# DiltheyLab/MetaMaps

Hardware: AMD Instinct MI355X
Metric: Gbp long reads mapped+classified per sec (whole node), miniSeq+H DB (higher is better)
Workload: dtype u32

## Files before the change

### include/metamaps_hip.h

```cpp
#ifndef METAMAPS_HIP_H
#define METAMAPS_HIP_H

#include <stddef.h>
#include <stdint.h>

#ifdef __cplusplus
extern "C" {
#endif

#define MM_ABI_VERSION 6

typedef enum {
  MM_OK = 0,
  MM_ERR_ARG = -1,
  MM_ERR_DEVICE = -2,
  MM_ERR_NOMEM = -3,
  MM_ERR_STATE = -4,
  MM_ERR_LIMIT = -5,
  MM_ERR_NUMERIC = -6,
  MM_ERR_COMM = -7,
  MM_ERR_DATA = -8
} mm_status;

typedef struct mm_ctx mm_ctx;
// ... 135 lines not shown
  double ms_minimizer, ms_sketch, ms_probe_gather, ms_sort_hits, ms_l1_scan, ms_l2, ms_compact, ms_total, ms_hit_filter;
  int64_t n_reads_giant;
} mm_map_stats;

int mm_map_batch(mm_ctx* ctx, const mm_index* idx, const mm_seqset* reads, const mm_map_params* p, mm_mapping** out);
int mm_map_batch_phased(mm_ctx* ctx, const mm_index* idx, const mm_seqset* reads, const mm_map_params* p, void (*at_stage)(void* user, int stage), void* user,
                        mm_mapping** out);
int mm_map_batch_reusing(mm_ctx* ctx, const mm_index* idx, const mm_seqset* reads, const mm_map_params* p, const mm_mapping* sketch_of, mm_mapping** out);
int mm_sketch_batch(mm_ctx* ctx, const mm_seqset* reads, const mm_map_params* p, mm_mapping** out);
void mm_mapping_destroy(mm_mapping* m);
int mm_mapping_get_stats(const mm_mapping* m, mm_map_stats* out);
int mm_mapping_release_intermediates(mm_mapping* m);
int mm_mapping_fetch(mm_mapping* m, int64_t* offsets, mm_map_record* records, int64_t cap);
int mm_mapping_add_qualities(mm_ctx* ctx, mm_mapping* m, const mm_seqset* reads, int k);
int mm_mapping_keep_best(mm_ctx* ctx, mm_mapping* m, int k);
int mm_mapping_concat(mm_ctx* ctx, mm_mapping* const* parts, const int32_t* contig_base, int n_parts, mm_mapping** out);
int mm_mapping_from_parts(mm_ctx* ctx, int64_t n_reads, const int32_t* read_len, const mm_map_params* p, int n_parts,
                          const int64_t* const* offsets, const mm_map_record* const* records, const int32_t* contig_base, mm_mapping** out);

int mm_mapping_gather(mm_ctx* ctx, int owner, int64_t n_reads, const int32_t* read_len, const mm_map_params* p, mm_mapping* const* parts, const int32_t* chunk_id,
                      int n_parts, int n_chunks, const int32_t* chunk_rank, const int32_t* contig_base, mm_mapping** out);

int mm_debug_sketch(mm_mapping* m, int64_t* offsets, uint32_t* hash, int32_t* strand, int64_t cap);
int mm_debug_hits(mm_mapping* m, int64_t* offsets, int32_t* contig, int32_t* wpos, int64_t cap);
int mm_debug_candidates(mm_mapping* m, int64_t* offsets, int32_t* triples , int64_t cap);
int mm_debug_l2(mm_mapping* m, int64_t* per_cand , int64_t cap);
int mm_debug_min_hits(mm_mapping* m, int32_t* min_hits );
int mm_debug_probed_lists(mm_mapping* m, const mm_index* idx, int64_t* hist, int32_t n_bins);

int mm_em_create(mm_ctx* ctx, int64_t n_reads, const int64_t* read_off, const int32_t* taxon, const double* mapq,
                 const double* inv_nloc, int32_t n_taxa, mm_em** out);
int mm_em_create_from_mapping(mm_ctx* ctx, const mm_mapping* m, const int32_t* contig_taxon, const int32_t* contig_len, int32_t n_contigs,
                              int32_t n_taxa, mm_em** out);
int mm_em_taxon_counts(mm_em* em, int64_t* counts);
int mm_em_sizes(const mm_em* em, int64_t* n_reads, int64_t* n_entries, int32_t* n_taxa);
void mm_em_destroy(mm_em* em);
int mm_em_iterate(mm_em* em, const double* f, double* f_partial, double* ll_partial);
int mm_em_iterate_allreduce(mm_em* em, const double* f, double* f_next, double* ll);
int mm_em_run(mm_em* em, const double* f0, int max_iter, double* f_out, double* ll_trace, int ll_cap, int* n_iter);
int mm_em_continue(mm_em* em, int max_iter, double* f_out, double* ll_trace, int ll_cap, int* n_iter, int* stopped);
int mm_em_posteriors(mm_em* em, const double* f, double* post , int64_t* best );
int mm_em_bootstrap(mm_em* em, const double* f_start, int32_t rep0, int32_t n_rep, uint64_t seed, const uint8_t* weights,
                    int max_iter, double* f_out, double* ll_out, int32_t* n_iter, int32_t* stopped);
int mm_em_lca(mm_em* em, const double* f, int32_t n_nodes, const int32_t* parent, const int32_t* taxon_node, double threshold,
              int32_t* node_out, double* mass_out, int64_t* direct_out);

// ... 27 lines not shown
```

### metamaps_amd/capi.py

```python
from __future__ import annotations

import ctypes as C
import os
import re

import numpy as np

_HERE = os.path.dirname(os.path.abspath(__file__))
LIB_PATH = os.path.join(_HERE, "csrc", "libmetamaps_hip.so")
HEADER_PATH = os.path.join(os.path.dirname(_HERE), "include", "metamaps_hip.h")

COMM_ID_BYTES = 128
MM_ERR_ARG = -1
MM_ERR_LIMIT = -5
MM_ERR_DATA = -8


class MMError(RuntimeError):
    def __init__(self, status: int, msg: str):
        super().__init__(f"libmetamaps_hip status {status}: {msg}")
        self.status = status


SEED_STAGE_CB = C.CFUNCTYPE(None, C.c_void_p, C.c_int)
# ... 119 lines not shown
            "mm_index_set_freq_threshold": (C.c_int, [vp, C.c_int]),
            "mm_index_entries": (C.c_int, [vp, vp, vp, vp, vp, i64]),
            "mm_index_dup_neighbours": (C.c_int, [vp, vp, vp, i64]),
            "mm_recommended_window": (C.c_int, [f64, C.c_int, f32, C.c_int, u64]),
            "mm_estimate_pvalue": (f64, [C.c_int, C.c_int, f32, C.c_int, u64]),
            "mm_min_hits_relaxed": (C.c_int, [C.c_int, C.c_int, f32]),
            "mm_identity": (None, [C.c_int, C.c_int, C.c_int, P(f32), P(f32)]),
            "mm_map_batch": (C.c_int, [vp, vp, vp, P(MapParams), P(vp)]),
            "mm_map_batch_phased": (C.c_int, [vp, vp, vp, P(MapParams), SEED_STAGE_CB, vp, P(vp)]),
            "mm_map_batch_reusing": (C.c_int, [vp, vp, vp, P(MapParams), vp, P(vp)]),
            "mm_sketch_batch": (C.c_int, [vp, vp, P(MapParams), P(vp)]),
            "mm_mapping_destroy": (None, [vp]),
            "mm_mapping_get_stats": (C.c_int, [vp, P(MapStats)]),
            "mm_comm_info": (C.c_int, [vp, C.POINTER(C.c_int), C.POINTER(C.c_int)]),
            "mm_mapping_gather": (C.c_int, [vp, C.c_int, i64, vp, vp, vp, vp, C.c_int, C.c_int, vp, vp, vp]),
            "mm_mapping_release_intermediates": (C.c_int, [vp]),
            "mm_mapping_fetch": (C.c_int, [vp, vp, vp, i64]),
            "mm_mapping_add_qualities": (C.c_int, [vp, vp, vp, C.c_int]),
            "mm_mapping_concat": (C.c_int, [vp, P(vp), vp, C.c_int, P(vp)]),
            "mm_mapping_keep_best": (C.c_int, [vp, vp, C.c_int]),
            "mm_mapping_from_parts": (C.c_int, [vp, i64, vp, P(MapParams), C.c_int, P(vp), P(vp), vp, P(vp)]),
            "mm_index_plan_chunks": (C.c_int, [vp, vp, u64, vp, i32, P(i32)]),
            "mm_debug_sketch": (C.c_int, [vp, vp, vp, vp, i64]),
            "mm_debug_hits": (C.c_int, [vp, vp, vp, vp, i64]),
            "mm_debug_candidates": (C.c_int, [vp, vp, vp, i64]),
            "mm_debug_l2": (C.c_int, [vp, vp, i64]),
            "mm_debug_min_hits": (C.c_int, [vp, vp]),
            "mm_debug_probed_lists": (C.c_int, [vp, vp, vp, i32]),
            "mm_em_create": (C.c_int, [vp, i64, vp, vp, vp, vp, i32, P(vp)]),
            "mm_em_create_from_mapping": (C.c_int, [vp, vp, vp, vp, i32, i32, P(vp)]),
            "mm_em_taxon_counts": (C.c_int, [vp, vp]),
            "mm_em_sizes": (C.c_int, [vp, P(i64), P(i64), P(i32)]),
            "mm_em_destroy": (None, [vp]),
            "mm_em_iterate": (C.c_int, [vp, vp, vp, P(f64)]),
            "mm_em_iterate_allreduce": (C.c_int, [vp, vp, vp, P(f64)]),
            "mm_em_posteriors": (C.c_int, [vp, vp, vp, vp]),
            "mm_em_run": (C.c_int, [vp, vp, C.c_int, vp, vp, C.c_int, P(C.c_int)]),
            "mm_em_continue": (C.c_int, [vp, C.c_int, vp, vp, C.c_int, P(C.c_int), P(C.c_int)]),
            "mm_em_bootstrap": (C.c_int, [vp, vp, i32, i32, u64, vp, C.c_int, vp, vp, vp, vp]),
            "mm_em_lca": (C.c_int, [vp, vp, i32, vp, vp, f64, vp, vp, vp]),
            "mm_gene_overlap": (C.c_int, [vp, i32, vp, vp, vp, vp, i32, vp, vp, i32, i64, vp, vp, vp, vp, vp, vp, vp, P(i64)]),
            "mm_ident_filter": (C.c_int, [vp, i64, vp, vp, vp, vp, i32, f64, vp, P(i64), P(i64), vp, vp, vp, vp, vp, vp, vp, P(i64), P(i64)]),
            "mm_comm_unique_id": (C.c_int, [C.c_char_p]),
            "mm_comm_init": (C.c_int, [vp, C.c_char_p, C.c_int, C.c_int]),
            "mm_comm_allreduce_f64": (C.c_int, [vp, vp, i64]),
            "mm_comm_share": (C.c_int, [vp, vp]),
            "mm_comm_destroy": (None, [vp]),
        }
        for name, (res, args) in sig.items():
            fn = getattr(L, name)
            fn.restype = res
            fn.argtypes = args
        _lib = L
    return _lib


def _ptr(a):
    return None if a is None else a.ctypes.data_as(C.c_void_p)


class Context:
    def __init__(self, device: int = 0):
        self.h = C.c_void_p()
        st = lib().mm_ctx_create(device, C.byref(self.h))
        if st != 0:
            raise MMError(st, "mm_ctx_create failed (no gfx950 GPU visible? this library has no CPU fallback)")

    def check(self, st: int):
        if st != 0:
            raise MMError(st, lib().mm_last_error(self.h).decode(errors="replace"))

    def close(self):
# ... 454 lines not shown
        arr = (C.c_void_p * max(len(parts), 1))(*[p.h for p in parts])
        cid = np.asarray(chunk_id, dtype=np.int32); crk = np.asarray(chunk_rank, dtype=np.int32); base = np.asarray(contig_base, dtype=np.int32)
        mp = MapParams(k, w, pi, min_read_len)
        out = C.c_void_p()
        ctx.check(lib().mm_mapping_gather(ctx.h, owner, len(rl), _ptr(rl), C.byref(mp), arr, _ptr(cid), len(parts), len(crk), _ptr(crk), _ptr(base), C.byref(out)))
        return Mapping(ctx, out, len(rl)) if out.value else None

    def fetch(self, rec_buf: np.ndarray | None = None):
        off = np.empty(self.n_reads + 1, dtype=np.int64)
        self.ctx.check(lib().mm_mapping_fetch(self.h, _ptr(off), None, 0))
        n = int(off[-1])
        rec = rec_buf[:n] if rec_buf is not None and len(rec_buf) >= n else np.empty(n, dtype=RECORD_DTYPE)
        self.ctx.check(lib().mm_mapping_fetch(self.h, _ptr(off), _ptr(rec), n))
        return off, rec

    def debug_sketch(self):
        off = np.zeros(self.n_reads + 1, dtype=np.int64)
        self.ctx.check(lib().mm_debug_sketch(self.h, _ptr(off), None, None, 0))
        h = np.zeros(int(off[-1]), dtype=np.uint32)
        s = np.zeros(int(off[-1]), dtype=np.int32)
        self.ctx.check(lib().mm_debug_sketch(self.h, _ptr(off), _ptr(h), _ptr(s), len(h)))
        return off, h, s

    def debug_hits(self):
        off = np.zeros(self.n_reads + 1, dtype=np.int64)
        self.ctx.check(lib().mm_debug_hits(self.h, _ptr(off), None, None, 0))
        c = np.zeros(int(off[-1]), dtype=np.int32)
        w = np.zeros(int(off[-1]), dtype=np.int32)
        self.ctx.check(lib().mm_debug_hits(self.h, _ptr(off), _ptr(c), _ptr(w), len(c)))
        return off, c, w

    def debug_candidates(self):
        off = np.zeros(self.n_reads + 1, dtype=np.int64)
        self.ctx.check(lib().mm_debug_candidates(self.h, _ptr(off), None, 0))
        t = np.zeros((int(off[-1]), 3), dtype=np.int32)
        self.ctx.check(lib().mm_debug_candidates(self.h, _ptr(off), _ptr(t), len(t)))
        return off, t

    def debug_l2(self, n_cand: int):
        a = np.zeros((n_cand, 6), dtype=np.int64)
        if n_cand:
            self.ctx.check(lib().mm_debug_l2(self.h, _ptr(a), n_cand))
        return a

    def debug_min_hits(self):
        a = np.zeros(self.n_reads, dtype=np.int32)
# ... 94 lines not shown
```

### metamaps_amd/csrc/mm_api.hip

```cpp
#include "mm_env.hpp"
#include "mm_map.hpp"
#include "mm_em.hpp"
#include "mm_stats.hpp"
#include "mm_synth.hpp"
#include "mm_hpc.hpp"
#include "mm_lca.hpp"
#include "mm_gene.hpp"
#include "mm_ident.hpp"
#include <chrono>
#include <new>
#include <rccl/rccl.h>
#include "mm_prims.hpp"

namespace mm {
void seqset_upload(mm_seqset* s);
void seqset_upload_nt16(mm_seqset* s);
int64_t bgzf_inflate(mm_ctx* ctx, const uint8_t* comp, int64_t comp_bytes, const int64_t* comp_off, const int32_t* comp_len, int32_t n,
                     uint8_t* out, int64_t out_cap, const int64_t* out_off, int32_t* status);
void bgzf_deflate(mm_ctx* ctx, const uint8_t* in, int64_t in_bytes, uint8_t* out, int64_t out_cap, int64_t* out_bytes, int32_t* n_blocks);
int64_t bgzf_deflate_bound(int64_t in_bytes);
mm_gzip* gzip_open(mm_ctx* ctx, int64_t chunk, int64_t segment);
void gzip_close(mm_gzip* g);
int gzip_feed(mm_gzip* g, const uint8_t* comp, int64_t n, bool last, int64_t* avail);
int64_t gzip_read(mm_gzip* g, uint8_t* out, int64_t cap);
// ... 748 lines not shown
  });
}

int mm_debug_sketch(mm_mapping* m, int64_t* offsets, uint32_t* hash, int32_t* strand, int64_t cap) {
  if (m && m->released) return MM_ERR_STATE;
  if (!m) return MM_ERR_ARG;
  return guarded(m->ctx, [&] {
    hipStream_t st = m->ctx->stream;
    int64_t tot = 0;
    for (int64_t r = 0; r < m->n_reads; ++r) { if (offsets) offsets[r] = tot; tot += m->h_sk_n[(size_t)r]; }
    if (offsets) offsets[m->n_reads] = tot;
    if (!hash && !strand) return;
    MM_REQUIRE(cap >= tot, MM_ERR_ARG, "output capacity too small");
    auto hh = m->sk_hash.to_host(st); auto hs = m->sk_strand.to_host(st);
    int64_t o = 0;
    for (int64_t r = 0; r < m->n_reads; ++r)
      for (int i = 0; i < m->h_sk_n[(size_t)r]; ++i, ++o) {
        size_t src = (size_t)m->mz.h_off[(size_t)r] + (size_t)i;
        if (hash) hash[o] = hh[src];
        if (strand) strand[o] = (hs[src] & 1) ? 1 : -1;
      }
  });
}
int mm_debug_hits(mm_mapping* m, int64_t* offsets, int32_t* contig, int32_t* wpos, int64_t cap) {
  if (m && m->released) return MM_ERR_STATE;
  if (!m) return MM_ERR_ARG;
  return guarded(m->ctx, [&] {
    const int64_t tot = (int64_t)m->h_read_hit_off[(size_t)m->n_reads];
    if (offsets) for (size_t i = 0; i < m->h_read_hit_off.size(); ++i) offsets[i] = (int64_t)m->h_read_hit_off[i];
    if (!contig && !wpos) return;
    MM_REQUIRE(cap >= tot, MM_ERR_ARG, "output capacity too small");
    auto h = m->hits.to_host(m->ctx->stream, (size_t)tot);
    for (int64_t i = 0; i < tot; ++i) {
      if (contig) contig[i] = (int32_t)(h[(size_t)i] >> 32);
      if (wpos) wpos[i] = mm::pw_wpos((uint32_t)h[(size_t)i]);
    }
  });
}
int mm_debug_candidates(mm_mapping* m, int64_t* offsets, int32_t* triples, int64_t cap) {
  if (m && m->released) return MM_ERR_STATE;
  if (!m) return MM_ERR_ARG;
  return guarded(m->ctx, [&] {
    if (offsets) for (size_t i = 0; i < m->h_cand_off.size(); ++i) offsets[i] = (int64_t)m->h_cand_off[i];
    if (!triples) return;
    MM_REQUIRE(cap >= m->n_cand, MM_ERR_ARG, "output capacity too small");
    m->cand.download(triples, (size_t)(3 * m->n_cand), m->ctx->stream);
// ... 169 lines not shown
```

### metamaps_amd/csrc/mm_env.hpp

```cpp
#pragma once
#include <unistd.h>
#include <cstdlib>
#include <cstring>
#include <string>

extern "C" char** environ;

namespace mm {

struct EnvSwitch { const char* name; const char* dflt; const char* kind; const char* what; };

inline const EnvSwitch* env_table(size_t* n) {
  static const EnvSwitch T[] = {
    {"MM_STRICT_ENV", "unset", "user", "refuse MM_* variables that are not in this table (mm_ctx_create returns MM_ERR_ARG, the CLI exits 1)"},
    {"MM_CPU_BUDGET", "min(hardware threads, affinity mask, cgroup CPU quota)", "user", "CPUs the process may keep busy: what every thread pool of the library and the CLI is sized from (cpu_budget.hpp)"},
    {"MM_SYNC", "block when the CPU budget is <= 32, else spin", "user", "how a host thread waits for its stream: \"spin\" (hipStreamSynchronize) or \"block\" (sleep on an event created with hipEventBlockingSync)"},
    {"MM_CLI_WORKERS", "4", "user", "worker contexts per GPU that take read batches in turn (= --workers-per-gpu)"},
    {"MM_CLI_BATCH_READS", "100000", "user", "reads per batch handed to a worker"},
    {"MM_CLI_BATCH_MBASES", "256", "user", "... or this many million bases, whichever comes first"},
    {"MM_CLI_MAP_SLOTS", "2", "tuning", "batches per device that may be inside their mapping section at the same time"},
    {"MM_CLI_BLOCK_BYTES", "128 MiB", "tuning", "block size of the block-parallel FASTQ/FASTA parser over an mmap-ed query file"},
    {"MM_CLI_REF_BLOCK_BYTES", "min(group, 256 MiB)", "tuning", "the same for the reference FASTA"},
    {"MM_CLI_REF_GROUP_BASES", "2^30", "test", "bases per upload group of the reference (small groups: the concat path on small inputs)"},
    {"MM_CLI_REF_SEQUENTIAL", "unset", "test", "reference through the sequential kseq-style reader instead of the block parser"},
// ... 6 lines not shown
    {"MM_DEFLATE_HOST", "unset", "test", "mm_bgzf_deflate (the mappings file of --compress-output) writes its BGZF members with zlib level 1 on the host's threads instead of the device kernel: the A/B partner and a fallback; other bytes, the same text"},
    {"MM_CLI_NO_PREWARM", "unset", "test", "worker contexts come up with their first batch instead of beside the index build"},
    {"MM_SF_GRID", "the device's CU count", "debug", "resident workgroups of the streaming seed filter (measurement aid: how K3 scales with the CUs at work)"},
    {"MM_CLI_LATE_READER", "unset", "debug", "the query reader starts when the index is built instead of beside the build (measurement aid)"},
    {"MM_CLI_NO_SKETCH_REUSE", "unset", "test", "chunk-major runs recompute minimizers and sketches per chunk (mm_map_batch instead of mm_map_batch_reusing)"},
    {"MM_CLI_NO_HUGE", "unset", "test", "no transparent-huge-page arena for host blocks >= 4 MiB (huge_new.hpp)"},
    {"MM_CLI_FULL_TEARDOWN", "unset", "test", "destroy every object and run static destructors at exit instead of _exit after the last file is closed"},
    {"MM_CLASSIFY_THREADS", "32", "user", "host threads that tokenise the mappings file and format classify's outputs"},
    {"MM_EM_MAX_ITER", "unbounded", "test", "cap on EM iterations in classify (the reference has none)"},
    {"MM_EM_SLICE", "1024", "test", "EM iterations per mm_em_run / mm_em_continue call of classify"},
    {"MM_CLI_TIMING", "unset", "debug", "phase laps of the CLI on stderr (bench.py's e2e legs parse them)"},
    {"MM_CLI_FORMAT_TRACE", "unset", "debug", "per-thread times of the text formatting of a batch on stderr"},
    {"MM_DEVICE_BYTES_CAP", "0 (off)", "test", "the library behaves as if every device had this many bytes: allocations beyond fail, mm_ctx_device_info reports it (placement tests)"},
    {"MM_INDEX_SCALE_MB", "8192", "test", "blocks from this size on are index-scale (pooled per device); a few MB exercise the pool on small inputs"},
    {"MM_NO_SLABS", "unset", "test", "worker buffers are not cut out of pooled index-scale blocks"},
    {"MM_NO_POOL_RESCUE", "unset", "test", "round-3 behaviour: a request the driver refuses hands the whole pool back instead of being served from it"},
    {"MM_ALLOC_TRACE", "unset", "debug", "every block that comes from the driver, with its cost, on stderr"},
    {"MM_CTX_TRACE", "unset", "debug", "phases of mm_ctx_create (HIP initialisation, stream, allocator) on stderr"},
    {"MM_HOST_TIMING", "unset", "debug", "host-side sections of mm_map_batch and of the index build on stderr"},
    {"MM_PACK_SCALAR", "unset", "test", "mm_seqset_upload packs bases with the byte-table loop only (cross-check of the AVX2 path, host_pack.cpp)"},
    {"MM_INDEX_PART_MAX", "2^31 - 2^24 entries", "test", "entries per partition of the hash sort (small values: the partitioned sort + merge on small inputs)"},
    {"MM_DUP_SAT", "65535", "test", "saturation value of the stored same-hash neighbour distances (small values: K5's scan fall-back)"},
    {"MM_EAGER_TIEBREAK", "unset", "test", "resolve every duplicate-hash strand by the reference's std::sort order up front instead of only where a strand vote reads one"},
    {"MM_FORCE_AMB_REDO", "unset", "test", "every read with an unresolved strand goes through the redo path"},
    {"MM_NO_HIT_FILTER", "unset", "test", "K3 without the exact seed-hit pre-filter: every hit of every kept list reaches the sort (parity tests of the raw hit list)"},
    {"MM_NO_FUSED_FILTER", "unset", "test", "K3 as probe_kernel + two-pass hit_filter_kernel for every read (what reads that do not fit the fused kernel take)"},
    {"MM_HF_STAGE_CAP", "auto", "test", "capacity of a read's survivor stage (tiny values: the overflow / re-filter path)"},
    {"MM_HF_WIDE_FROM", "13000", "tuning", "sketch size from which the two-pass filter counts in 32768 position slots instead of 8192"},
    {"MM_SEGSORT_MAX_KEYS", "2^32 - 1", "test", "keys per call of K4's segmented device sort (small values: the split on small inputs)"},
    {"MM_L1_SERIAL", "unset", "test", "K4's L1 merge loop as the literal one-thread-per-read loop (cross-check of the wavefront form)"},
    {"MM_L2_FULL", "unset", "test", "K5 evaluates every window (the literal slide) instead of the exact skip-ahead"},
    {"MM_L2_DENSE_FROM", "13000", "tuning", "sketch size from which K5 runs as l2_codes_kernel + l2_dense_kernel"},
    {"MM_L2_DENSE_NO_STOP", "unset", "test", "dense path without its early stop (every window evaluated)"},
    {"MM_L2_NO_SMALL_GROUPS", "unset", "test", "groups of fewer than three candidates also run as four-wave workgroups (one launch instead of two)"},
    {"MM_L2_HOST_GROUPS", "unset", "test", "candidate groups formed on the host instead of by l2_group_kernel"},
    {"MM_L2_NO_GROUP_SORT", "unset", "test", "K5 workgroups in read order instead of the order of their candidates' positions"},
    {"MM_L2_GROUP_SORT_MIN", "2048", "tuning", "groups from which the launch order is sorted"},
    {"MM_L2_V1", "unset", "test", "K5's 10 kb class through l2_kernel (rank codes per entry) instead of the zone kernel l2z_kernel (mm_l2z.hpp): the cross-check and the A/B"},
    {"MM_L2_V1_LONG", "unset", "test", "the long-read classes (sketches of 3 073 .. 13 000 hashes) through l2_kernel, the 10 kb class through the zone kernel"},
    {"MM_L2_NO_FUSE", "unset", "test", "zone kernel without the band predicted from L1's seed-hit count: its masks always come from a second pass over the stream"},
    {"MM_L2_NO_RANGES", "unset", "test", "the zone kernel's waves search their candidates' index ranges themselves (until round 6) instead of taking them from l2_ranges_kernel (cross-check)"},
    {"MM_L2Z_FORCE_HANDBACK", "unset", "test", "the zone kernel hands every candidate that reaches its band loop to l2_kernel, as its pass-count guard does (the hand-back path against the default)"},
    {"MM_L2Z_WALK_SEARCH", "unset", "test", "the 10 kb zone kernel finds the next block to sweep by the walk one block at a time (the long-read classes' way) instead of by ballots: the same blocks, the cross-check"},
    {"MM_L2Z_DBG", "unset", "debug", "zone kernel writes pivot-minus-estimate and its pass count INSTEAD OF RESULTS (tools/l2z_pivot_hist.py; 2: against the predicted estimate)"},
    {"MM_L2_ONE_STREAM", "unset", "test", "the two launches of K5's 10 kb class one behind the other on the context's stream instead of side by side (auxiliary stream)"},
    {"MM_L2_NO_SLOTS", "unset", "test", "K5 scratch indexed by wave number of the launch instead of per-XCD slots taken and given back"},
// ... 40 lines not shown
```

### metamaps_amd/csrc/mm_map.hip

```cpp
#include "mm_map.hpp"
#include <functional>
#include <memory>
#include "mm_prims.hpp"
#include "mm_l2_core.hpp"
#include "mm_size_classes.hpp"
#include "mm_l2.hpp"
#include "mm_l2z.hpp"
#include "mm_l2_dense.hpp"
#include <cstdlib>
#include <atomic>
#include <thread>
#include "mm_stats.hpp"
#include <algorithm>
#include <numeric>
#include "mm_sketch.hpp"
#include "mm_seed.hpp"
#include "mm_l1.hpp"

namespace mm {

namespace {
struct HostLap {
  const bool on = getenv("MM_HOST_TIMING") != nullptr; std::chrono::steady_clock::time_point t = std::chrono::steady_clock::now();
  void operator()(const char* what) { if (!on) return; const auto n = std::chrono::steady_clock::now(); fprintf(stderr, "host %-28s %8.1f us\n", what, std::chrono::duration<double, std::micro>(n - t).count()); t = n; }
// ... 37 lines not shown
  void end(size_t i) { MM_HIP(hipEventRecord(ev[i].second, st)); }
  void collect() {
    MM_HIP(mm::stream_sync(st));
    for (size_t i = 0; i < ev.size(); ++i) { float ms = 0; MM_HIP(hipEventElapsedTime(&ms, ev[i].first, ev[i].second)); *dst[i] += ms; }
  }
};
}

struct AmbState {
  std::thread bg;
  std::vector<Rec> hr; std::vector<uint64_t> dof; std::vector<int32_t> expect; DBuf<uint64_t> d_so, d_do;
  std::vector<uint8_t> sv; std::vector<int32_t> scnt; std::atomic<int> mismatch{0};
  ~AmbState() { if (bg.joinable()) bg.join(); }
};

namespace {
struct MapSwitches {
  struct OptInt { bool set; int v; };
  static bool on(const char* e) { return e != nullptr; }
  static bool is1(const char* e) { return e && e[0] == '1'; }
  static int num(const char* e, int dflt) { return e ? atoi(e) : dflt; }
  static OptInt opt(const char* e) { return OptInt{e != nullptr, e ? atoi(e) : 0}; }
  const bool eager_tiebreak = on(getenv("MM_EAGER_TIEBREAK"));
  const bool use_filter = !is1(getenv("MM_NO_HIT_FILTER"));
  const bool use_fused = use_filter && !on(getenv("MM_NO_FUSED_FILTER"));
  const int hf_wide_env = num(getenv("MM_HF_WIDE_FROM"), 13000);
  const int hf_wide_from = hf_wide_env > 0 ? hf_wide_env : INT_MAX;
  const OptInt hf_stage_cap = opt(getenv("MM_HF_STAGE_CAP"));
  const int hf_dbg = num(getenv("MM_HF_DBG"), 0);
  const bool sf_prof = on(getenv("MM_SF_PROF"));
  const OptInt sf_grid = opt(getenv("MM_SF_GRID"));
  const OptInt segsort_max_env = opt(getenv("MM_SEGSORT_MAX_KEYS"));
  const uint64_t segsort_max_keys = segsort_max_env.set ? (uint64_t)std::max(segsort_max_env.v, 1) : 0xffffffffull;
  const bool l1_serial = on(getenv("MM_L1_SERIAL"));
  const bool l2_no_fuse = on(getenv("MM_L2_NO_FUSE"));
  const bool l2_no_ranges = on(getenv("MM_L2_NO_RANGES"));
  const bool l2_skip = !is1(getenv("MM_L2_FULL"));
  const int dense_from = num(getenv("MM_L2_DENSE_FROM"), 13000);
  const bool dense_no_stop = on(getenv("MM_L2_DENSE_NO_STOP"));
  const bool no_small_groups = on(getenv("MM_L2_NO_SMALL_GROUPS"));
  const bool dev_groups = l2_skip && !on(getenv("MM_L2_HOST_GROUPS"));
  const bool l2_no_slots = on(getenv("MM_L2_NO_SLOTS"));
  const OptInt l2_slots_env = opt(getenv("MM_L2_SLOTS"));
  const size_t l2_slots = l2_slots_env.set ? ((size_t)std::max(l2_slots_env.v, 1) + 7) / 8 * 8 : 0;
  const bool v2 = !on(getenv("MM_L2_V1"));
  const bool v2_long = v2 && !on(getenv("MM_L2_V1_LONG"));
// ... 129 lines not shown
    size_t t_sk = T.begin(&M->stats.ms_sketch);
    static_assert(ipt_list_is<4, 6, 8, 10, 12, 16, 20, 24, 32, 40, 48, 64>(SKETCH_IPTS), "the dispatch below lists the classes of mm_size_classes.hpp");
    uint64_t big_seen = 0;
    HostLap hl;
    const ReadBins RB = bin_reads(n, N_SKETCH_CLASSES, [&](int64_t r) -> int {
      const uint64_t c = hoff()[(size_t)r + 1] - hoff()[(size_t)r];
      big_seen |= (uint64_t)(c > SKETCH_LDS_MAX);
      return sketch_class_index(c);
    });
    const bool any_big = big_seen != 0;
    {
      hl("K2 bin");
      DBuf<int32_t> list(std::max<size_t>(RB.order.size(), 1));
      list.upload(RB.order.data(), RB.order.size(), st);
      hl("K2 list upload");
      size_t at = 0;
      for (auto& run : RB.runs) {
        const unsigned nb = (unsigned)run.second;
        const int32_t* lp = list.p + at;
        dispatch<4, 6, 8, 10, 12, 16, 20, 24, 32, 40, 48, 64>(SKETCH_IPTS[run.first], [&](auto ipt_tag) {
          constexpr int IPT = decltype(ipt_tag)::value;
          using SortT = rocprim::block_radix_sort<uint32_t, 256, IPT, uint16_t>;
          using ScanT = rocprim::block_scan<int, 256>;
          const size_t lds = std::max(sizeof(typename SortT::storage_type), sizeof(typename ScanT::storage_type)) + 16;
          if (lds > 48 * 1024) MM_HIP(hipFuncSetAttribute((const void*)sketch_radix_kernel<IPT>, hipFuncAttributeMaxDynamicSharedMemorySize, (int)lds));
          sketch_radix_kernel<IPT><<<dim3(nb), dim3(256), lds, st>>>(M->mz.rec.p, M->mz.off.p, lp, M->sk_hash.p, M->sk_strand.p, M->sk_n.p, M->amb.p);
        });
        MM_KERNEL_CHECK();
        at += run.second;
      }
      hl("K2 launches");
      MM_HIP(mm::stream_sync(st));
      hl("K2 sync (kernels)");
    }
    if (any_big) sketch_big_segmented();
    T.end(t_sk);
  }

  void sketch_big_segmented() {
    std::vector<int32_t> big; std::vector<uint64_t> koff{0};
    for (int64_t r = 0; r < n; ++r) { const uint64_t c = hoff()[(size_t)r + 1] - hoff()[(size_t)r]; if (c > SKETCH_LDS_MAX) { big.push_back((int32_t)r); koff.push_back(koff.back() + c); } }
    const size_t nb = big.size(); const uint64_t nk = koff.back();
    MM_REQUIRE(nk < ((uint64_t)1 << 32), MM_ERR_LIMIT, "more than 2^32 minimizers of reads beyond 16384 minimizers in one batch");
    DBuf<int32_t> d_big(nb); d_big.upload(big.data(), nb, st);
    DBuf<uint64_t> d_koff(nb + 1); d_koff.upload(koff.data(), nb + 1, st);
    DBuf<uint64_t> keys((size_t)nk), sorted((size_t)nk);
    sketch_keys_kernel<<<dim3((unsigned)nb), dim3(256), 0, st>>>(M->mz.rec.p, M->mz.off.p, d_big.p, d_koff.p, keys.p);
    MM_KERNEL_CHECK();
    DBuf<uint8_t> tmp;
// ... 717 lines not shown
```

### metamaps_amd/csrc/mm_minimizer.hpp

```cpp
#pragma once
#include <type_traits>
#include "mm_common.hpp"
#include "mm_scan.hpp"

namespace mm {

constexpr int MZ_THREADS = 256;
constexpr int MZ_TILE = 2048;
constexpr int MZ_MAX_W = 4096;
constexpr int MZ_STAGE = 1024;
constexpr int MZ_MAX_K = 64;

struct SeqView {
  const uint32_t* packed;
  const uint64_t* base;
  const int32_t* len;
  const uint64_t* exc_start;
  const uint32_t* exc_len;
  const uint8_t* exc_byte;
  int64_t n_exc;
  int64_t n;
};

__device__ inline uint32_t code_at(const SeqView& S, uint64_t g) { return (S.packed[g >> 4] >> (2 * (g & 15))) & 3u; }

__device__ inline int64_t exc_lower(const SeqView& S, uint64_t g) {
// ... 199 lines not shown
    for (int j = jeval0 + tid; j < hb8; j += MZ_THREADS) {
      uint16_t c = 0xFFFF;
      if (flg[j] & 1) {
        uint32_t best = hsh[j]; int bj = j;
        const int qlo = max(j - w + 1, 0);
        for (int q = j - 1; q >= qlo; --q)
          if ((flg[q] & 1) && hsh[q] < best) { best = hsh[q]; bj = q; }
        c = (uint16_t)bj;
      }
      cps[j] = c;
    }
    for (int g = (hb8 >> 3) + tid; g * 8 < np; g += MZ_THREADS) {
      uint32_t h[16]; uint8_t f[16];
      {
        const uint4 a = g ? *reinterpret_cast<const uint4*>(hsh + 8 * g - 8) : make_uint4(0, 0, 0, 0);
        const uint4 b = g ? *reinterpret_cast<const uint4*>(hsh + 8 * g - 4) : make_uint4(0, 0, 0, 0);
        const uint4 c = *reinterpret_cast<const uint4*>(hsh + 8 * g), d = *reinterpret_cast<const uint4*>(hsh + 8 * g + 4);
        h[0] = a.x; h[1] = a.y; h[2] = a.z; h[3] = a.w; h[4] = b.x; h[5] = b.y; h[6] = b.z; h[7] = b.w;
        h[8] = c.x; h[9] = c.y; h[10] = c.z; h[11] = c.w; h[12] = d.x; h[13] = d.y; h[14] = d.z; h[15] = d.w;
        const uint64_t fa = g ? *reinterpret_cast<const uint64_t*>(flg + 8 * g - 8) : 0ull, fb = *reinterpret_cast<const uint64_t*>(flg + 8 * g);
#pragma unroll
        for (int t = 0; t < 8; ++t) { f[t] = (uint8_t)(fa >> (8 * t)); f[8 + t] = (uint8_t)(fb >> (8 * t)); }
      }
      uint64_t key[16];
#pragma unroll
      for (int t = 0; t < 16; ++t) key[t] = (f[t] & 1) ? ((uint64_t)h[t] << 8) | (uint64_t)(255 - t) : ~0ull;
      uint64_t res[8];
      auto mn = [](uint64_t a, uint64_t b) { return a < b ? a : b; };
      auto windows = [&](auto wtag) {
        constexpr int W = decltype(wtag)::value;
        uint64_t m1[16], m2[16], m4[16];
#pragma unroll
        for (int t = 1; t < 16; ++t) m1[t] = mn(key[t], key[t - 1]);
#pragma unroll
        for (int t = 3; t < 16; ++t) m2[t] = mn(m1[t], m1[t - 2]);
#pragma unroll
        for (int t = 7; t < 16; ++t) m4[t] = mn(m2[t], m2[t - 4]);
#pragma unroll
        for (int i = 0; i < 8; ++i) {
          const int t = 8 + i;
          if constexpr (W == 1) res[i] = key[t];
          else if constexpr (W == 2) res[i] = m1[t];
          else if constexpr (W == 3) res[i] = mn(m1[t], m1[t - 1]);
          else if constexpr (W == 4) res[i] = m2[t];
          else if constexpr (W < 8) res[i] = mn(m2[t], m2[t - (W - 4)]);
          else if constexpr (W == 8) res[i] = m4[t];
          else res[i] = mn(m4[t], m4[t - 1]);
        }
      };
      switch (w) {
        case 1: windows(std::integral_constant<int, 1>{}); break;
        case 2: windows(std::integral_constant<int, 2>{}); break;
        case 3: windows(std::integral_constant<int, 3>{}); break;
        case 4: windows(std::integral_constant<int, 4>{}); break;
        case 5: windows(std::integral_constant<int, 5>{}); break;
        case 6: windows(std::integral_constant<int, 6>{}); break;
        case 7: windows(std::integral_constant<int, 7>{}); break;
        case 8: windows(std::integral_constant<int, 8>{}); break;
        default: windows(std::integral_constant<int, 9>{}); break;
      }
#pragma unroll
      for (int i = 0; i < 8; ++i) {
        const int j = 8 * g + i;
        if (j < jeval0 || j >= np) continue;
        cps[j] = (f[8 + i] & 1) ? (uint16_t)(8 * g - 8 + 255 - (int)(res[i] & 0xffu)) : (uint16_t)0xFFFF;
      }
    }
  } else
  for (int j = jeval0 + tid; j < np; j += MZ_THREADS) {
    uint16_t c = 0xFFFF;
    if (flg[j] & 1) {
      uint32_t best = hsh[j]; int bj = j;
      const int qlo = max(j - w + 1, 0);
      for (int q = j - 1; q >= qlo; --q)
        if ((flg[q] & 1) && hsh[q] < best) { best = hsh[q]; bj = q; }
      c = (uint16_t)bj;
    }
    cps[j] = c;
  }
  __syncthreads();
  if (dbgs == 3) { if (MODE != 1 && tid == 0) tile_count[tile] = 0; return; }
  const int js = jstar[s];
  const int j0 = (P0 - H0) + tid * (MZ_TILE / MZ_THREADS);
  uint32_t mask = 0;
  static_assert(MZ_TILE / MZ_THREADS == 8, "eight positions per thread");
  bool fast = false;
  if (w >= 2 && j0 + 8 <= np && H0 + j0 - 1 >= w - 1 && j0 >= 1) {
    const uint2 fw = *reinterpret_cast<const uint2*>(flg + j0);
// ... 77 lines not shown
```

### metamaps_amd/csrc/mm_sketch.hpp

```cpp
#pragma once
#include <rocprim/rocprim.hpp>
#include "mm_map.hpp"

namespace mm {

template <int IPT>
__global__ void __launch_bounds__(256) sketch_radix_kernel(const Rec* __restrict__ rec, const uint64_t* __restrict__ off,
                                                           const int32_t* __restrict__ read_list, uint32_t* __restrict__ sk_hash,
                                                           uint8_t* __restrict__ sk_strand, int32_t* __restrict__ sk_n, uint8_t* __restrict__ amb) {
  using Sort = rocprim::block_radix_sort<uint32_t, 256, IPT, uint16_t>;
  using Scan = rocprim::block_scan<int, 256>;
  union Tmp { typename Sort::storage_type sort; typename Scan::storage_type scan; };
  extern __shared__ __align__(16) unsigned char sketch_dyn[];
  Tmp& tmp = *reinterpret_cast<Tmp*>(sketch_dyn);
  __shared__ uint32_t last_key[256];
  __shared__ uint8_t last_st[256];
  __shared__ int s_amb;
  const int r = read_list[blockIdx.x];
  const uint64_t o = off[r];
  const int n = (int)(off[r + 1] - o);
  const int t = threadIdx.x;
  uint32_t key[IPT]; uint16_t val[IPT];
#pragma unroll
  for (int i = 0; i < IPT; ++i) { const int idx = t * IPT + i; key[i] = idx < n ? rec[o + idx].hash : 0xffffffffu; val[i] = (uint16_t)idx; }
  if (t == 0) s_amb = 0;
  Sort().sort(key, val, tmp.sort);
  uint8_t stv[IPT];
#pragma unroll
  for (int i = 0; i < IPT; ++i) stv[i] = (t * IPT + i < n) ? (uint8_t)(rec[o + val[i]].pw & PW_STRAND) : 0;
  last_key[t] = key[IPT - 1]; last_st[t] = stv[IPT - 1];
  __syncthreads();
  int nfirst = 0; bool first[IPT]; bool ambig = false;
#pragma unroll
  for (int i = 0; i < IPT; ++i) {
    const int pos = t * IPT + i;
    const uint32_t pk = i ? key[i - 1] : (t ? last_key[t - 1] : 0u);
    const uint8_t ps = i ? stv[i - 1] : (t ? last_st[t - 1] : 0);
    first[i] = pos < n && (pos == 0 || pk != key[i]);
    if (pos < n && pos > 0 && pk == key[i] && ps != stv[i]) ambig = true;
    nfirst += first[i] ? 1 : 0;
  }
  if (ambig) s_amb = 1;
  int ex = 0, total = 0;
  Scan().exclusive_scan(nfirst, ex, 0, total, tmp.scan);
  const int ex0 = ex;
#pragma unroll
  for (int i = 0; i < IPT; ++i) if (first[i]) { sk_hash[o + ex] = key[i]; sk_strand[o + ex] = stv[i]; ++ex; }
  __threadfence_block();
  __syncthreads();
  if (s_amb) {
    int ex2 = ex0;
#pragma unroll
    for (int i = 0; i < IPT; ++i) {
      const int pos = t * IPT + i;
      if (first[i]) ++ex2;
      const uint32_t pk = i ? key[i - 1] : (t ? last_key[t - 1] : 0u);
      const uint8_t ps = i ? stv[i - 1] : (t ? last_st[t - 1] : 0);
      if (pos < n && pos > 0 && pk == key[i] && ps != stv[i]) sk_strand[o + ex2 - 1] |= 2;
    }
  }
  if (t == 0) { sk_n[r] = total; amb[r] = (uint8_t)(s_amb ? 2 : 0); }
}

__global__ void __launch_bounds__(256) sketch_keys_kernel(const Rec* __restrict__ rec, const uint64_t* __restrict__ off, const int32_t* __restrict__ read_list,
                                                          const uint64_t* __restrict__ koff, uint64_t* __restrict__ keys) {
  const int r = read_list[blockIdx.x];
  const uint64_t o = off[r], k0 = koff[blockIdx.x];
  const uint32_t n = (uint32_t)(off[r + 1] - o);
  for (uint32_t i = threadIdx.x; i < n; i += 256) keys[k0 + i] = ((uint64_t)rec[o + i].hash << 32) | i;
}
__global__ void __launch_bounds__(256) sketch_finish_kernel(const Rec* __restrict__ rec, const uint64_t* __restrict__ off, const int32_t* __restrict__ read_list,
                                                            const uint64_t* __restrict__ koff, const uint64_t* __restrict__ sorted,
                                                            uint32_t* __restrict__ sk_hash, uint8_t* __restrict__ sk_strand, int32_t* __restrict__ sk_n, uint8_t* __restrict__ amb) {
  const int r = read_list[blockIdx.x];
  const uint64_t o = off[r];
  const uint64_t* __restrict__ a = sorted + koff[blockIdx.x];
  const int n = (int)(off[r + 1] - o);
  __shared__ int s_amb;
  if (threadIdx.x == 0) s_amb = 0;
  __syncthreads();
  for (int pass = 0; pass < 2; ++pass) {
    uint64_t carry = 0;
    for (int base = 0; base < n; base += 256) {
      const int i = base + threadIdx.x;
// ... 44 lines not shown
```

Baseline: 26.33.

## Replace per-read minimizer radix sort with one-pass bucket sort and argmin windows

Reads of up to 4096 minimizers are now sketched by a new bucket kernel instead of a block radix sort. It counts hashes into LDS buckets, scatters them, and ranks each element within its small bucket. Then it dedups and marks ambiguous strands with wave ballots. Reads whose buckets overflow fall back to the radix path. Separately, the 64-bit packed-key window minimum in minimizer selection is replaced by a 32-bit (hash, slot) argmin using prefix/suffix combines. The trade-off is extra LDS per block and occupancy pressure, plus new debug API surface.

```diff
diff --git a/include/metamaps_hip.h b/include/metamaps_hip.h
--- a/include/metamaps_hip.h
+++ b/include/metamaps_hip.h
@@ -181,6 +181,7 @@
                       int n_parts, int n_chunks, const int32_t* chunk_rank, const int32_t* contig_base, mm_mapping** out);
 
 int mm_debug_sketch(mm_mapping* m, int64_t* offsets, uint32_t* hash, int32_t* strand, int64_t cap);
+int mm_debug_sketch_marks(mm_mapping* m, uint8_t* strand_bytes, uint8_t* amb , int64_t cap);
 int mm_debug_hits(mm_mapping* m, int64_t* offsets, int32_t* contig, int32_t* wpos, int64_t cap);
 int mm_debug_candidates(mm_mapping* m, int64_t* offsets, int32_t* triples , int64_t cap);
 int mm_debug_l2(mm_mapping* m, int64_t* per_cand , int64_t cap);
diff --git a/metamaps_amd/capi.py b/metamaps_amd/capi.py
--- a/metamaps_amd/capi.py
+++ b/metamaps_amd/capi.py
@@ -165,6 +165,7 @@
             "mm_mapping_from_parts": (C.c_int, [vp, i64, vp, P(MapParams), C.c_int, P(vp), P(vp), vp, P(vp)]),
             "mm_index_plan_chunks": (C.c_int, [vp, vp, u64, vp, i32, P(i32)]),
             "mm_debug_sketch": (C.c_int, [vp, vp, vp, vp, i64]),
+            "mm_debug_sketch_marks": (C.c_int, [vp, vp, vp, i64]),
             "mm_debug_hits": (C.c_int, [vp, vp, vp, vp, i64]),
             "mm_debug_candidates": (C.c_int, [vp, vp, vp, i64]),
             "mm_debug_l2": (C.c_int, [vp, vp, i64]),
@@ -191,6 +192,8 @@
             "mm_comm_destroy": (None, [vp]),
         }
         for name, (res, args) in sig.items():
+            if name == "mm_debug_sketch_marks" and not hasattr(L, name):
+                continue
             fn = getattr(L, name)
             fn.restype = res
             fn.argtypes = args
@@ -691,6 +694,14 @@
         self.ctx.check(lib().mm_debug_sketch(self.h, _ptr(off), _ptr(h), _ptr(s), len(h)))
         return off, h, s
 
+    def debug_sketch_marks(self):
+        off = np.zeros(self.n_reads + 1, dtype=np.int64)
+        self.ctx.check(lib().mm_debug_sketch(self.h, _ptr(off), None, None, 0))
+        b = np.zeros(int(off[-1]), dtype=np.uint8)
+        amb = np.zeros(self.n_reads, dtype=np.uint8)
+        self.ctx.check(lib().mm_debug_sketch_marks(self.h, _ptr(b), _ptr(amb), len(b)))
+        return b, amb
+
     def debug_hits(self):
         off = np.zeros(self.n_reads + 1, dtype=np.int64)
         self.ctx.check(lib().mm_debug_hits(self.h, _ptr(off), None, None, 0))
diff --git a/metamaps_amd/csrc/mm_api.hip b/metamaps_amd/csrc/mm_api.hip
--- a/metamaps_amd/csrc/mm_api.hip
+++ b/metamaps_amd/csrc/mm_api.hip
@@ -794,6 +794,23 @@
       }
   });
 }
+int mm_debug_sketch_marks(mm_mapping* m, uint8_t* strand_bytes, uint8_t* amb, int64_t cap) {
+  if (m && m->released) return MM_ERR_STATE;
+  if (!m) return MM_ERR_ARG;
+  return guarded(m->ctx, [&] {
+    hipStream_t st = m->ctx->stream;
+    if (strand_bytes) {
+      int64_t tot = 0;
+      for (int64_t r = 0; r < m->n_reads; ++r) tot += m->h_sk_n[(size_t)r];
+      MM_REQUIRE(cap >= tot, MM_ERR_ARG, "output capacity too small");
+      auto hs = m->sk_strand.to_host(st);
+      int64_t o = 0;
+      for (int64_t r = 0; r < m->n_reads; ++r)
+        for (int i = 0; i < m->h_sk_n[(size_t)r]; ++i, ++o) strand_bytes[o] = hs[(size_t)m->mz.h_off[(size_t)r] + (size_t)i];
+    }
+    if (amb) { auto ha = m->amb.to_host(st, (size_t)m->n_reads); for (int64_t r = 0; r < m->n_reads; ++r) amb[r] = ha[(size_t)r]; }
+  });
+}
 int mm_debug_hits(mm_mapping* m, int64_t* offsets, int32_t* contig, int32_t* wpos, int64_t cap) {
   if (m && m->released) return MM_ERR_STATE;
   if (!m) return MM_ERR_ARG;
diff --git a/metamaps_amd/csrc/mm_env.hpp b/metamaps_amd/csrc/mm_env.hpp
--- a/metamaps_amd/csrc/mm_env.hpp
+++ b/metamaps_amd/csrc/mm_env.hpp
@@ -52,6 +52,7 @@
     {"MM_INDEX_PART_MAX", "2^31 - 2^24 entries", "test", "entries per partition of the hash sort (small values: the partitioned sort + merge on small inputs)"},
     {"MM_DUP_SAT", "65535", "test", "saturation value of the stored same-hash neighbour distances (small values: K5's scan fall-back)"},
     {"MM_EAGER_TIEBREAK", "unset", "test", "resolve every duplicate-hash strand by the reference's std::sort order up front instead of only where a strand vote reads one"},
+    {"MM_SKETCH_RADIX", "unset", "test", "K2 sorts every read's minimizers with sketch_radix_kernel; by default reads of at most 4 096 minimizers take the one-pass sketch_bucket_kernel (cross-check and the A/B)"},
     {"MM_FORCE_AMB_REDO", "unset", "test", "every read with an unresolved strand goes through the redo path"},
     {"MM_NO_HIT_FILTER", "unset", "test", "K3 without the exact seed-hit pre-filter: every hit of every kept list reaches the sort (parity tests of the raw hit list)"},
     {"MM_NO_FUSED_FILTER", "unset", "test", "K3 as probe_kernel + two-pass hit_filter_kernel for every read (what reads that do not fit the fused kernel take)"},
diff --git a/metamaps_amd/csrc/mm_map.hip b/metamaps_amd/csrc/mm_map.hip
--- a/metamaps_amd/csrc/mm_map.hip
+++ b/metamaps_amd/csrc/mm_map.hip
@@ -83,6 +83,7 @@
   static int num(const char* e, int dflt) { return e ? atoi(e) : dflt; }
   static OptInt opt(const char* e) { return OptInt{e != nullptr, e ? atoi(e) : 0}; }
   const bool eager_tiebreak = on(getenv("MM_EAGER_TIEBREAK"));
+  const bool sketch_radix = on(getenv("MM_SKETCH_RADIX"));
   const bool use_filter = !is1(getenv("MM_NO_HIT_FILTER"));
   const bool use_fused = use_filter && !on(getenv("MM_NO_FUSED_FILTER"));
   const int hf_wide_env = num(getenv("MM_HF_WIDE_FROM"), 13000);
@@ -258,9 +259,15 @@
           constexpr int IPT = decltype(ipt_tag)::value;
           using SortT = rocprim::block_radix_sort<uint32_t, 256, IPT, uint16_t>;
           using ScanT = rocprim::block_scan<int, 256>;
-          const size_t lds = std::max(sizeof(typename SortT::storage_type), sizeof(typename ScanT::storage_type)) + 16;
-          if (lds > 48 * 1024) MM_HIP(hipFuncSetAttribute((const void*)sketch_radix_kernel<IPT>, hipFuncAttributeMaxDynamicSharedMemorySize, (int)lds));
-          sketch_radix_kernel<IPT><<<dim3(nb), dim3(256), lds, st>>>(M->mz.rec.p, M->mz.off.p, lp, M->sk_hash.p, M->sk_strand.p, M->sk_n.p, M->amb.p);
+          size_t lds = std::max(sizeof(typename SortT::storage_type), sizeof(typename ScanT::storage_type)) + 16;
+          auto launch = [&](auto kernel) {
+            if (lds > 48 * 1024) MM_HIP(hipFuncSetAttribute((const void*)kernel, hipFuncAttributeMaxDynamicSharedMemorySize, (int)lds));
+            kernel<<<dim3(nb), dim3(256), lds, st>>>(M->mz.rec.p, M->mz.off.p, lp, M->sk_hash.p, M->sk_strand.p, M->sk_n.p, M->amb.p);
+          };
+          if constexpr (IPT <= SKB_MAX_IPT) {
+            if (!sw.sketch_radix) { lds = std::max(lds, sketch_bucket_lds_bytes<IPT>()); launch(sketch_bucket_kernel<IPT>); return; }
+          }
+          launch(sketch_radix_kernel<IPT>);
         });
         MM_KERNEL_CHECK();
         at += run.second;
diff --git a/metamaps_amd/csrc/mm_minimizer.hpp b/metamaps_amd/csrc/mm_minimizer.hpp
--- a/metamaps_amd/csrc/mm_minimizer.hpp
+++ b/metamaps_amd/csrc/mm_minimizer.hpp
@@ -2,6 +2,7 @@
 #include <type_traits>
 #include "mm_common.hpp"
 #include "mm_scan.hpp"
+#include "mm_minimizer_core.hpp"
 
 namespace mm {
 
@@ -247,10 +248,14 @@
 #pragma unroll
         for (int t = 0; t < 8; ++t) { f[t] = (uint8_t)(fa >> (8 * t)); f[8 + t] = (uint8_t)(fb >> (8 * t)); }
       }
+#ifndef MZ_ARGMIN64
+      uint32_t slot[8];
+      mz_argmin8(h, f, w, slot);
+#else
       uint64_t key[16];
 #pragma unroll
       for (int t = 0; t < 16; ++t) key[t] = (f[t] & 1) ? ((uint64_t)h[t] << 8) | (uint64_t)(255 - t) : ~0ull;
-      uint64_t res[8];
+      uint64_t res[8]; uint32_t slot[8];
       auto mn = [](uint64_t a, uint64_t b) { return a < b ? a : b; };
       auto windows = [&](auto wtag) {
         constexpr int W = decltype(wtag)::value;
@@ -285,10 +290,13 @@
         default: windows(std::integral_constant<int, 9>{}); break;
       }
 #pragma unroll
+      for (int i = 0; i < 8; ++i) slot[i] = 255u - (uint32_t)(res[i] & 0xffu);
+#endif
+#pragma unroll
       for (int i = 0; i < 8; ++i) {
         const int j = 8 * g + i;
         if (j < jeval0 || j >= np) continue;
-        cps[j] = (f[8 + i] & 1) ? (uint16_t)(8 * g - 8 + 255 - (int)(res[i] & 0xffu)) : (uint16_t)0xFFFF;
+        cps[j] = (f[8 + i] & 1) ? (uint16_t)(8 * g - 8 + (int)slot[i]) : (uint16_t)0xFFFF;
       }
     }
   } else
diff --git a/metamaps_amd/csrc/mm_minimizer_core.hpp b/metamaps_amd/csrc/mm_minimizer_core.hpp
--- /dev/null
+++ b/metamaps_amd/csrc/mm_minimizer_core.hpp
@@ -0,0 +1,77 @@
+#pragma once
+#include <stdint.h>
+
+#ifndef MM_HD
+#if defined(__HIPCC__)
+#define MM_HD __host__ __device__ inline
+#else
+#define MM_HD inline
+#endif
+#endif
+
+#if defined(__clang__)
+#define MM_UNROLL _Pragma("unroll")
+#else
+#define MM_UNROLL
+#endif
+
+namespace mm {
+
+struct MzPair { uint32_t h, s; };
+MM_HD MzPair mz_combine(const MzPair a, const MzPair b) {
+  const bool right = b.h <= a.h;
+  return MzPair{right ? b.h : a.h, right ? b.s : a.s};
+}
+
+template <int W>
+MM_HD void mz_argmin8_w(const uint32_t* h, const uint8_t* ns, uint32_t* slot) {
+  static_assert(W >= 1 && W <= 9, "a window reaches at most eight slots back");
+  MzPair e[16];
+  MM_UNROLL
+  for (int t = 0; t < 16; ++t) e[t] = MzPair{(ns[t] & 1) ? h[t] : 0xffffffffu, (uint32_t)t};
+  if constexpr (W >= 8) {
+    MzPair suf[8], pre[16];
+    suf[7] = e[7];
+    MM_UNROLL
+    for (int t = 6; t >= 9 - W; --t) suf[t] = mz_combine(e[t], suf[t + 1]);
+    pre[8] = e[8];
+    MM_UNROLL
+    for (int t = 9; t < 16; ++t) pre[t] = mz_combine(pre[t - 1], e[t]);
+    MM_UNROLL
+    for (int i = 0; i < 8; ++i) {
+      const int t = 8 + i, from = t - W + 1;
+      slot[i] = (from >= 8 ? pre[t] : mz_combine(suf[from], pre[t])).s;
+    }
+  } else {
+    MzPair m1[16], m2[16];
+    MM_UNROLL
+    for (int t = 1; t < 16; ++t) m1[t] = mz_combine(e[t - 1], e[t]);
+    MM_UNROLL
+    for (int t = 3; t < 16; ++t) m2[t] = mz_combine(m1[t - 2], m1[t]);
+    MM_UNROLL
+    for (int i = 0; i < 8; ++i) {
+      const int t = 8 + i;
+      if constexpr (W == 1) slot[i] = e[t].s;
+      else if constexpr (W == 2) slot[i] = m1[t].s;
+      else if constexpr (W == 3) slot[i] = mz_combine(m1[t - 1], m1[t]).s;
+      else if constexpr (W == 4) slot[i] = m2[t].s;
+      else slot[i] = mz_combine(m2[t - (W - 4)], m2[t]).s;
+    }
+  }
+}
+
+MM_HD void mz_argmin8(const uint32_t* h, const uint8_t* ns, int w, uint32_t* slot) {
+  switch (w) {
+    case 1: mz_argmin8_w<1>(h, ns, slot); break;
+    case 2: mz_argmin8_w<2>(h, ns, slot); break;
+    case 3: mz_argmin8_w<3>(h, ns, slot); break;
+    case 4: mz_argmin8_w<4>(h, ns, slot); break;
+    case 5: mz_argmin8_w<5>(h, ns, slot); break;
+    case 6: mz_argmin8_w<6>(h, ns, slot); break;
+    case 7: mz_argmin8_w<7>(h, ns, slot); break;
+    case 8: mz_argmin8_w<8>(h, ns, slot); break;
+    default: mz_argmin8_w<9>(h, ns, slot); break;
+  }
+}
+
+}
diff --git a/metamaps_amd/csrc/mm_sketch.hpp b/metamaps_amd/csrc/mm_sketch.hpp
--- a/metamaps_amd/csrc/mm_sketch.hpp
+++ b/metamaps_amd/csrc/mm_sketch.hpp
@@ -1,24 +1,20 @@
 #pragma once
 #include <rocprim/rocprim.hpp>
 #include "mm_map.hpp"
+#include "mm_sketch_core.hpp"
 
 namespace mm {
 
-template <int IPT>
-__global__ void __launch_bounds__(256) sketch_radix_kernel(const Rec* __restrict__ rec, const uint64_t* __restrict__ off,
-                                                           const int32_t* __restrict__ read_list, uint32_t* __restrict__ sk_hash,
-                                                           uint8_t* __restrict__ sk_strand, int32_t* __restrict__ sk_n, uint8_t* __restrict__ amb) {
+template <int IPT, bool OVERFLOW_BRANCH>
+__device__ inline void sketch_radix_read(unsigned char* sketch_dyn, const Rec* __restrict__ rec, const uint64_t o, const int n, const int r, uint32_t* __restrict__ sk_hash,
+                                         uint8_t* __restrict__ sk_strand, int32_t* __restrict__ sk_n, uint8_t* __restrict__ amb) {
   using Sort = rocprim::block_radix_sort<uint32_t, 256, IPT, uint16_t>;
   using Scan = rocprim::block_scan<int, 256>;
   union Tmp { typename Sort::storage_type sort; typename Scan::storage_type scan; };
-  extern __shared__ __align__(16) unsigned char sketch_dyn[];
   Tmp& tmp = *reinterpret_cast<Tmp*>(sketch_dyn);
   __shared__ uint32_t last_key[256];
   __shared__ uint8_t last_st[256];
   __shared__ int s_amb;
-  const int r = read_list[blockIdx.x];
-  const uint64_t o = off[r];
-  const int n = (int)(off[r + 1] - o);
   const int t = threadIdx.x;
   uint32_t key[IPT]; uint16_t val[IPT];
 #pragma unroll
@@ -60,6 +56,144 @@
     }
   }
   if (t == 0) { sk_n[r] = total; amb[r] = (uint8_t)(s_amb ? 2 : 0); }
+}
+template <int IPT>
+__global__ void __launch_bounds__(256) sketch_radix_kernel(const Rec* __restrict__ rec, const uint64_t* __restrict__ off,
+                                                           const int32_t* __restrict__ read_list, uint32_t* __restrict__ sk_hash,
+                                                           uint8_t* __restrict__ sk_strand, int32_t* __restrict__ sk_n, uint8_t* __restrict__ amb) {
+  extern __shared__ __align__(16) unsigned char sketch_dyn[];
+  const int r = read_list[blockIdx.x];
+  const uint64_t o = off[r];
+  sketch_radix_read<IPT, false>(sketch_dyn, rec, o, (int)(off[r + 1] - o), r, sk_hash, sk_strand, sk_n, amb);
+}
+
+__device__ inline int block_excl_scan_i32(int v, int* total) {
+  __shared__ int wsum[4];
+  const int lane = threadIdx.x & 63, wid = threadIdx.x >> 6;
+  int inc = v;
+#pragma unroll
+  for (int d = 1; d < 64; d <<= 1) { const int o = __shfl_up(inc, d, 64); if (lane >= d) inc += o; }
+  if (lane == 63) wsum[wid] = inc;
+  __syncthreads();
+  int base = 0, tot = 0;
+#pragma unroll
+  for (int i = 0; i < 4; ++i) { if (i < wid) base += wsum[i]; tot += wsum[i]; }
+  __syncthreads();
+  *total = tot;
+  return base + inc - v;
+}
+
+template <int IPT>
+constexpr size_t sketch_bucket_lds_bytes() { return ((size_t)skb_buckets(IPT) + 4) * 4 + (size_t)256 * IPT * (6 + 5); }
+template <int IPT>
+__global__ void __launch_bounds__(256) __attribute__((amdgpu_waves_per_eu(4))) sketch_bucket_kernel(const Rec* __restrict__ rec, const uint64_t* __restrict__ off,
+                                                            const int32_t* __restrict__ read_list, uint32_t* __restrict__ sk_hash,
+                                                            uint8_t* __restrict__ sk_strand, int32_t* __restrict__ sk_n, uint8_t* __restrict__ amb) {
+  static_assert(IPT <= SKB_MAX_IPT, "the tag holds 12 index bits");
+  constexpr int CAP = 256 * IPT, BITS = skb_bucket_bits(IPT), NB = 1 << BITS, CPT = NB / 256;
+  static_assert(CPT % 4 == 0, "the scan reads its counters four at a time");
+  extern __shared__ __align__(16) unsigned char sketch_dyn[];
+  uint32_t* const start = reinterpret_cast<uint32_t*>(sketch_dyn);
+  uint32_t* const H = start + NB + 4;
+  uint32_t* const H2 = H + CAP;
+  uint16_t* const TG = reinterpret_cast<uint16_t*>(H2 + CAP);
+  uint8_t* const ST = reinterpret_cast<uint8_t*>(TG);
+  uint8_t* const ST2 = reinterpret_cast<uint8_t*>(TG + CAP);
+  __shared__ int s_amb, s_wtot[4];
+  const int r = read_list[blockIdx.x];
+  const uint64_t o = off[r];
+  const int n = (int)(off[r + 1] - o);
+  const int t = threadIdx.x;
+#pragma unroll
+  for (int c = 0; c < CPT; ++c) start[c * 256 + t] = 0;
+  if (t == 0) s_amb = 0;
+  __syncthreads();
+  const uint2* __restrict__ rec2 = reinterpret_cast<const uint2*>(rec + o);
+  for (int base = 0; base < n; base += 1024) {
+    uint32_t h4[4];
+#pragma unroll
+    for (int j = 0; j < 4; ++j) { const int idx = base + j * 256 + t; h4[j] = idx < n ? rec2[idx].x : 0u; }
+#pragma unroll
+    for (int j = 0; j < 4; ++j) if (base + j * 256 + t < n) atomicAdd(&start[skb_bucket(h4[j], BITS)], 1u);
+  }
+  __syncthreads();
+  uint32_t cnt[CPT], sum = 0, fullest = 0;
+#pragma unroll
+  for (int c = 0; c < CPT; c += 4) {
+    const uint4 v = *reinterpret_cast<const uint4*>(start + t * CPT + c);
+    cnt[c] = v.x; cnt[c + 1] = v.y; cnt[c + 2] = v.z; cnt[c + 3] = v.w;
+  }
+#pragma unroll
+  for (int c = 0; c < CPT; ++c) { sum += cnt[c]; fullest = max(fullest, cnt[c]); }
+  if (__syncthreads_or(fullest > (uint32_t)SKB_BUCKET_CAP)) {
+    sketch_radix_read<IPT, true>(sketch_dyn, rec, o, n, r, sk_hash, sk_strand, sk_n, amb);
+    return;
+  }
+  int total;
+  uint32_t ex = (uint32_t)block_excl_scan_i32((int)sum, &total);
+#pragma unroll
+  for (int c = 0; c < CPT; ++c) { const uint32_t v = cnt[c]; cnt[c] = ex; ex += v; }
+#pragma unroll
+  for (int c = 0; c < CPT; c += 4) *reinterpret_cast<uint4*>(start + t * CPT + c) = make_uint4(cnt[c], cnt[c + 1], cnt[c + 2], cnt[c + 3]);
+  __syncthreads();
+  for (int base = 0; base < n; base += 1024) {
+    uint2 v4[4];
+#pragma unroll
+    for (int j = 0; j < 4; ++j) { const int idx = base + j * 256 + t; v4[j] = idx < n ? rec2[idx] : make_uint2(0u, 0u); }
+#pragma unroll
+    for (int j = 0; j < 4; ++j) {
+      const int idx = base + j * 256 + t;
+      if (idx < n) { const uint32_t p = atomicAdd(&start[skb_bucket(v4[j].x, BITS)], 1u); H[p] = v4[j].x; TG[p] = skb_tag((uint32_t)idx, v4[j].y & PW_STRAND); }
+    }
+  }
+  __syncthreads();
+  for (int p = t; p < n; p += 256) {
+    const uint32_t h = H[p]; const uint16_t tag = TG[p];
+    const int b = skb_bucket(h, BITS);
+    const uint32_t s = b ? start[b - 1] : 0u, e = start[b];
+    const uint32_t fp = s + (uint32_t)skb_rank_in_bucket(H, TG, (int)s, (int)e, h, tag);
+    H2[fp] = h; ST2[fp] = (uint8_t)(tag & 1u);
+  }
+  __syncthreads();
+  const int lane = t & 63, wv = t >> 6, p0 = wv * 64 * IPT;
+  const uint64_t below = ((uint64_t)1 << lane) - 1;
+  uint32_t firsts = 0, differs = 0; int wcount = 0;
+  for (int i = 0; i < IPT && p0 + i * 64 < n; ++i) {
+    const int pos = p0 + i * 64 + lane;
+    bool first = false, dif = false;
+    if (pos < n) {
+      const uint32_t h = H2[pos], st = ST2[pos], pk = pos ? H2[pos - 1] : 0u, ps = pos ? ST2[pos - 1] : 0u;
+      first = skb_first(pos, pk, h);
+      dif = skb_differs(pos, pk, ps, h, st);
+    }
+    firsts |= (first ? 1u : 0u) << i; differs |= (dif ? 1u : 0u) << i;
+    wcount += __popcll(__ballot(first));
+  }
+  if (differs) s_amb = 1;
+  if (lane == 0) s_wtot[wv] = wcount;
+  __syncthreads();
+  int wbase = 0; total = 0;
+#pragma unroll
+  for (int i = 0; i < 4; ++i) { if (i < wv) wbase += s_wtot[i]; total += s_wtot[i]; }
+  const bool any_amb = s_amb != 0;
+  int at = wbase;
+  for (int i = 0; i < IPT && p0 + i * 64 < n; ++i) {
+    const uint64_t fb = __ballot(firsts >> i & 1u);
+    if (firsts >> i & 1u) { const int pos = p0 + i * 64 + lane, e1 = at + __popcll(fb & below); H[e1] = H2[pos]; ST[e1] = ST2[pos]; }
+    at += __popcll(fb);
+  }
+  if (any_amb) {
+    __syncthreads();
+    at = wbase;
+    for (int i = 0; i < IPT && p0 + i * 64 < n; ++i) {
+      const uint64_t fb = __ballot(firsts >> i & 1u);
+      if (differs >> i & 1u) ST[at + __popcll(fb & below) - 1] |= 2;
+      at += __popcll(fb);
+    }
+  }
+  __syncthreads();
+  for (int j = t; j < total; j += 256) { sk_hash[o + j] = H[j]; sk_strand[o + j] = ST[j]; }
+  if (t == 0) { sk_n[r] = total; amb[r] = (uint8_t)(any_amb ? 2 : 0); }
 }
 
 __global__ void __launch_bounds__(256) sketch_keys_kernel(const Rec* __restrict__ rec, const uint64_t* __restrict__ off, const int32_t* __restrict__ read_list,
diff --git a/metamaps_amd/csrc/mm_sketch_core.hpp b/metamaps_amd/csrc/mm_sketch_core.hpp
--- /dev/null
+++ b/metamaps_amd/csrc/mm_sketch_core.hpp
@@ -0,0 +1,36 @@
+#pragma once
+#include <stdint.h>
+#include "mm_l2_core.hpp"
+
+namespace mm {
+
+constexpr int SKB_MAX_IPT = 16;
+constexpr int SKB_BUCKET_CAP = 32;
+
+constexpr int skb_bucket_bits(int ipt) {
+  int b = 0;
+  while ((2 << b) <= 256 * ipt) ++b;
+#ifdef SKB_MORE_BUCKETS
+  ++b;
+#endif
+  return b;
+}
+constexpr int skb_buckets(int ipt) { return 1 << skb_bucket_bits(ipt); }
+
+MM_HD int skb_bucket(uint32_t hash, int bucket_bits) { return l2_bucket(hash, 32 - bucket_bits); }
+
+MM_HD uint16_t skb_tag(uint32_t index, uint32_t strand_bit) { return (uint16_t)((index << 1) | (strand_bit & 1u)); }
+MM_HD bool skb_less(uint32_t ha, uint16_t ta, uint32_t hb, uint16_t tb) { return ha < hb || (ha == hb && ta < tb); }
+
+MM_HD int skb_rank_in_bucket(const uint32_t* h, const uint16_t* tag, int begin, int end, uint32_t hash, uint16_t mytag) {
+  int c = 0;
+  for (int j = begin; j < end; ++j) c += skb_less(h[j], tag[j], hash, mytag) ? 1 : 0;
+  return c;
+}
+
+MM_HD bool skb_first(int pos, uint32_t prev_hash, uint32_t hash) { return pos == 0 || prev_hash != hash; }
+MM_HD bool skb_differs(int pos, uint32_t prev_hash, uint32_t prev_strand, uint32_t hash, uint32_t strand) {
+  return pos > 0 && prev_hash == hash && prev_strand != strand;
+}
+
+}
```

Result: no change. 26.46 (median of 4 runs) (+0.5%).
